# jeong0982/gkr

Hardware: AMD Instinct MI355X
Metric: BN254-Fr sumcheck field-ops/sec @ 2^20 vars (higher is better)
Workload: dtype u32x8

## Files before the change

gkr_amd/csrc/capi_internal.h:

```cpp
#pragma once
#include <hip/hip_runtime.h>
#include <sched.h>
#include <stdio.h>
#include <stdlib.h>
#include <string.h>

#include <algorithm>
#include <chrono>
#include <condition_variable>
#include <map>
#include <memory>
#include <mutex>
#include <string>
#include <thread>
#include <vector>

#include "../../include/gkr_amd.h"
#include "fr64.h"
#include "host_cpus.h"
#include "hostpool.h"
#include "kernels.h"
#include "options.h"
#include "gate_seg.h"
#include "keccak.h"
// ... 54 lines not shown
        }
        gkr::gkr_ifma_init(canon);
        return true;
    }();
    return ready;
}

inline gkr::h64::F host_multi_hash(const gkr::h64::F* arr, int n, const gkr::h64::F* cts) {
    static const bool adx = !gkr::process_switch("GKR_NO_ADX") && gkr::gkr_adx_available();
    if (!adx) return gkr::h64::mimc7_multi_hash(arr, n, cts, nullptr);
    gkr::h64::F out;
    gkr::gkr_adx_multi_hash(reinterpret_cast<const uint64_t(*)[4]>(arr), n, reinterpret_cast<const uint64_t(*)[4]>(cts), out.l);
    return out;
}

constexpr int kHashChunkMax = 16;
constexpr int kMaxLayerK = GKR_MAX_K_NEXT, kMaxLayerKi = GKR_MAX_K_I, kMaxDenseK = GKR_MAX_K_NEXT_DEVICE_TRANSCRIPT;
inline void ifma_hash_chunk(const uint64_t (*vec)[3][4], const uint32_t* ln, int count, uint64_t (*out)[4]) {
    if (count > 8)
        gkr::gkr_ifma_multi_hash16(vec, ln, 3, out);
    else
        gkr::gkr_ifma_multi_hash8(vec, ln, 3, out);
}
inline int hash_chunk_size(int tables, int threads, int help_share = 0) {
    const long long forced = gkr::opt(gkr::OPT_hash_chunk);
    if (forced == 8 || forced == 16) return (int)forced;
    if (help_share > 1 && tables <= 3 * help_share) return 1;
    return tables >= 32 * threads ? 16 : 8;
}

inline hipError_t device_malloc(void** p, size_t bytes) { return hipMalloc(p, bytes); }
inline hipError_t device_free(void* p) { return hipFree(p); }

inline int default_host_threads() {
    if (const int v = gkr::process_int("GKR_HOST_THREADS", 0); v >= 1) return v;
    int cpus = usable_cpus();
    int local = 1;
    if (const int ranks = gkr::process_int("LOCAL_WORLD_SIZE", 1); ranks > 0) local = ranks;
    const int share = cpus / local;
    int t = share >= 6 ? share - 2 : (share >= 3 ? share - 1 : share);
    if (t < 1) t = 1;
    if (t > 64) t = 64;
    return t;
}

inline Fr to_dev(const gkr_fr& x) {
    Fr f;
    memcpy(&f, &x, 32);
    return f;
}

// ... 104 lines not shown
    std::vector<std::unique_ptr<PreparedCircuit>> circuits;
    hipStream_t stream = nullptr;
    hipStream_t aux = nullptr;
    hipStream_t late = nullptr;
    hipStream_t chain = nullptr;
    std::vector<hipEvent_t> aux_events;
    Fr* d_cts = nullptr;
    int transcript = GKR_TRANSCRIPT_HOST;
    std::string err;
    int profile = 0;
    std::map<std::string, ProfileRow> prof;
    std::vector<PendingEvent> pending;
    std::vector<hipEvent_t> event_pool;
    char name[256] = {0};
    uint32_t ticket = 0;
    std::unique_ptr<gkr::SpinPool> pool;
    std::unique_ptr<gkr::SpinPool> solo_pool;
    std::unique_ptr<AsyncWorker> copier;
    std::unique_ptr<AsyncWorker> liner;
    void* mle_arrivals_zeroed = nullptr;
    void* arrivals_zeroed = nullptr;
    void* gate_arrive_zeroed = nullptr;
    bool crew_member = false;
    int help_share = 0;
    int rounds_ahead = 0;
    std::unique_ptr<ProveCrew, void (*)(ProveCrew*)> crew{nullptr, nullptr};
    std::map<std::string, std::pair<void*, size_t>> ws;
    std::map<std::string, std::pair<void*, size_t>> pinned;

    hipError_t workspace(const char* slot, size_t bytes, void** out) {
        auto& e = ws[slot];
        if (e.second < bytes) {
            if (e.first) (void)device_free(e.first);
            e.first = nullptr;
            e.second = 0;
            hipError_t rc = device_malloc(&e.first, bytes);
            if (rc != hipSuccess) return rc;
            e.second = bytes;
        }
        *out = e.first;
        return hipSuccess;
    }
    hipError_t pinned_host(const char* slot, size_t bytes, void** out) {
        auto& e = pinned[slot];
        if (e.second < bytes) {
            if (e.first) (void)hipHostFree(e.first);
            e.first = nullptr;
// ... 148 lines not shown
        if (_e != hipSuccess) return (ctx)->hip_fail(_e, #expr); \
    } while (0)


namespace gkr_host {


template <typename T>
struct DevBuf {
    T* p = nullptr;
    ~DevBuf() {
        if (p) (void)hipFree(p);
    }
    hipError_t alloc(size_t count) { return hipMalloc(reinterpret_cast<void**>(&p), count * sizeof(T)); }
};

struct ThreadTimeAccount {
    double own_pieces_us = 0, helped_us = 0, spin_us = 0;
};
inline thread_local ThreadTimeAccount t_account;
struct HostAccountTotals {
    std::atomic<uint64_t> own_ns{0}, helped_ns{0}, spin_ns{0}, rest_ns{0}, lent_ns{0}, lent_idle_ns{0}, calls{0}, wake_ns{0};
    std::atomic<uint64_t> pieces{0}, piece_ns{0}, piece_pass_ns{0}, lanes[17] = {};
    std::atomic<bool> on{false};
};
inline HostAccountTotals& host_account_totals() {
    static HostAccountTotals t;
    return t;
}
inline bool accounting_on() { return host_account_totals().on.load(std::memory_order_relaxed); }
inline void account_piece(int transcripts, double pass_us, double total_us) {
    HostAccountTotals& t = host_account_totals();
    t.pieces.fetch_add(1, std::memory_order_relaxed);
    t.piece_ns.fetch_add((uint64_t)(total_us * 1e3), std::memory_order_relaxed);
    t.piece_pass_ns.fetch_add((uint64_t)(pass_us * 1e3), std::memory_order_relaxed);
    t.lanes[transcripts < 1 ? 1 : (transcripts > 16 ? 16 : transcripts)].fetch_add(1, std::memory_order_relaxed);
}
inline double now_us_dbg() { return std::chrono::duration<double, std::micro>(std::chrono::steady_clock::now().time_since_epoch()).count(); }

inline bool help_enabled() {
    static const bool on = !gkr::process_switch("GKR_NO_HELP");
    return on;
}
static void run_pieces(gkr::SpinPool* pool, const std::function<bool()>* work, bool several, int priority = 0) {
    auto run = [&] {
        if (pool)
            pool->run_now(work);
        else
            while ((*work)()) {
            }
    };
    const bool dbg = gkr::debug_timing() || accounting_on();
    const double t0 = dbg ? now_us_dbg() : 0.0;
    if (several && help_enabled()) {
        gkr::HelpBoard::Posted posted(work, priority);
        run();
    } else {
        run();
    }
    if (dbg) t_account.own_pieces_us += now_us_dbg() - t0;
}

template <typename Rec>
inline int wait_records(gkr_ctx* ctx, const volatile Rec* recs, int count, uint32_t ticket) {
    const auto t0 = std::chrono::steady_clock::now();
    const bool help = help_enabled();
    auto last_progress = t0;
    for (int b = 0; b < count; ++b) {
        uint32_t spins = 0, helped = 0;
        while (__atomic_load_n(&recs[b].seq, __ATOMIC_ACQUIRE) != ticket) {
            const bool dbg = gkr::debug_timing() || accounting_on();
            const double th0 = dbg ? now_us_dbg() : 0.0;
            const bool did_help = help && gkr::HelpBoard::instance().help();
            if (!did_help) GKR_CPU_RELAX();
            if (dbg) (did_help ? t_account.helped_us : t_account.spin_us) += now_us_dbg() - th0;
            if (did_help ? (++helped & 0x3F) == 0 : (++spins & 0xFFFF) == 0) {
                hipError_t q = hipStreamQuery(ctx->stream);
                if (q != hipSuccess && q != hipErrorNotReady) return ctx->hip_fail(q, "stream failed while waiting for a round");
                if (std::chrono::steady_clock::now() - last_progress > std::chrono::seconds(30)) {
                    if (q == hipSuccess && __atomic_load_n(&recs[b].seq, __ATOMIC_ACQUIRE) == ticket) break;
                    return ctx->fail(GKR_ERR_HIP, "timed out waiting for the device to publish a round");
                }
            }
        }
        if (spins | helped) last_progress = std::chrono::steady_clock::now();
    }
    return GKR_OK;
}

constexpr int kMaxGroups = 32;
constexpr int kMleShardTailLog2 = 6;

#define WS(ctx, slot, type, count, ptr) \
    HIP_TRY(ctx, (ctx)->workspace(slot, (size_t)(count) * sizeof(type), reinterpret_cast<void**>(&(ptr))))

inline int mle_pass_rounds(int m, int n, int jmax) {
// ... 119 lines not shown
```

gkr_amd/csrc/capi_layer.hip:

```cpp
#include "capi_internal.h"

namespace gkr_host {

void host_prod_pass_scalar(const uint64_t* recs, size_t rec_row_words, int count, int J, const uint32_t (*vec_len)[16],
                                  uint64_t (*c2)[16][4], uint64_t (*lin)[16][4], uint64_t (*c0)[16][4], uint64_t (*r)[16][4],
                                  uint64_t* weights, size_t w_row_words) {
    using namespace gkr::h64;
    const F* cts = host_mimc_constants64();
    const F one_m = to_mont(F{{1, 0, 0, 0}});
    for (int k = 0; k < count; ++k) {
        F M[64], SY[8], rm[gkr::kProdMaxJ];
        const F* rec = reinterpret_cast<const F*>(recs + (size_t)k * rec_row_words);
        const int n = 1 << J;
        for (int a = 0; a < n; ++a) {
            for (int b = 0; b < n; ++b) M[a * 8 + b] = rec[a * 8 + b];
            SY[a] = rec[64 + a];
        }
        for (int t = 0; t < J; ++t) {
            const int half = 1 << (J - t - 1);
            F p00 = M[0], p01 = M[half], p10 = M[half * 8], p11 = M[half * 8 + half], s0 = SY[0], s1 = SY[half];
            for (int x = 1; x < half; ++x) {
                p00 = add(p00, M[x * 8 + x]);
                p01 = add(p01, M[x * 8 + half + x]);
                p10 = add(p10, M[(half + x) * 8 + x]);
// ... 261 lines not shown
            gkr::launch_gate_rows_wide(R.span, k_i, k, R.g->plan, R.gate_eq(), R.eq, R.A, R.M, R.lb, R.item_partials, R.gate_arrive, R.s, R.sets, R.plan_counts,
                                       R.wu ? &wfuse : nullptr);
            c_tables_done = R.wu != nullptr;
        } else
            c_tables_done = gkr::launch_gate_rows(R.span, k_i, k, R.g->offsets, R.g->cursor, R.g->list, R.e_hi, R.e_lo, R.kl, R.eq, R.A, R.M, R.lb, &R.g->segs,
                                                  R.seg_partials, R.s, R.shard ? nullptr : &fuse, R.sets);
    }
    if (R.shard)
        if (const int rc = xch.sum(R.A, R.M, R.wlen, nullptr, GKR_OK)) return rc;
    if (!c_tables_done) gkr::launch_prod_c_setup(R.Wb, jp, P.pw, R.A, R.M, R.X, R.Y, k, (uint32_t)R.wlen, batch, R.s);
    return GKR_OK;
}

struct HostPass {
    const LayerPinned* pin;
    int batch, k;
    bool ifma;
    gkr_fr* const* out_coeffs;
    uint32_t* const* out_len;
    gkr_fr* const* out_r;
    uint32_t J, round0, tail_m, tail_jp;
    bool on_host;
    int chunk;
    std::atomic<int> next{0};
};

static bool host_pass_piece(HostPass& hp) {
    const LayerPinned& P = *hp.pin;
    const int first = hp.next.fetch_add(hp.chunk, std::memory_order_relaxed);
    if (first >= hp.batch) return false;
    const int cnt = hp.batch - first < hp.chunk ? hp.batch - first : hp.chunk;
    uint64_t c2[gkr::kProdMaxJ][16][4], lin[gkr::kProdMaxJ][16][4], c0[gkr::kProdMaxJ][16][4], rr[gkr::kProdMaxJ][16][4];
    uint32_t vl[gkr::kProdMaxJ][16];
    const bool acct = accounting_on();
    const double tp0 = acct ? now_us_dbg() : 0.0;
    if (hp.on_host)
        for (int i = 0; i < cnt; ++i)
            host_tail_pass(reinterpret_cast<gkr::h64::F*>(P.tail + (size_t)(first + i) * 3 * P.tail_stride()), P.tail_stride(), hp.tail_m, hp.tail_jp,
                           reinterpret_cast<const gkr::h64::F*>(P.pw + (size_t)(first + i) * 8), hp.J, reinterpret_cast<gkr::h64::F*>(&P.prec[first + i].v[0]));
    for (uint32_t t = 0; t < hp.J; ++t)
        for (int i = 0; i < cnt; ++i) vl[t][i] = 2u + (P.dep[(size_t)(first + i) * 32 + (hp.round0 + t) % hp.k] ? 1u : 0u);
    (hp.ifma && cnt >= 3 ? gkr::gkr_ifma_prod_pass : host_prod_pass_scalar)(
        reinterpret_cast<const uint64_t*>(P.prec + first), sizeof(gkr::ProdPassRec) / 8, cnt, (int)hp.J, vl, c2, lin, c0, rr,
        reinterpret_cast<uint64_t*>(P.pw + (size_t)first * 8), 32);
    const double tp1 = acct ? now_us_dbg() : 0.0;
    for (int i = 0; i < cnt; ++i) {
        const int b = first + i;
        for (uint32_t t = 0; t < hp.J; ++t) {
            const uint32_t round = hp.round0 + t;
            gkr_fr* oc = hp.out_coeffs[b] + (size_t)round * 3;
            memset(&oc[0], 0, 32);
            if (vl[t][i] == 3) memcpy(&oc[0], c2[t][i], 32);
            memcpy(&oc[1], lin[t][i], 32);
// ... 48 lines not shown
            const bool on_host = tail_active;
            const bool exports = P.tail && !on_host && m - jp <= P.tail_log2 && rem > J;
            if (!on_host) {
                const uint32_t ticket = ++ctx->ticket;
                const double tl0 = dbg_sections ? now_us_dbg() : 0.0;
                {
                    Timed t(ctx, "layer_prod_pass", 0.0);
                    gkr::launch_prod_pass(Tw, Tx, Ty, m, jp, P.pw, J, d_ppart, (uint32_t)R.wlen, P.prec, ticket, (uint32_t)batch, R.s, d_arrivals, d_fold_plans,
                                          exports ? P.tail : nullptr, (uint32_t)P.tail_stride());
                }
                if (hipError_t le = hipGetLastError(); le != hipSuccess) {
                    rc = ctx->hip_fail(le, "launch of a layer pass");
                    break;
                }
                const double tl1 = dbg_sections ? now_us_dbg() : 0.0;
                rc = wait_records(ctx, P.prec, batch, ticket);
                if (dbg_sections) {
                    us_launch += tl1 - tl0;
                    us_wait += now_us_dbg() - tl1;
                }
                if (!rc) rc = xch.check();
                if (rc) break;
            }
            const int chunk = hash_chunk_size(batch, pool ? pool->workers() + 1 : 1, ctx->crew_member ? ctx->help_share : 0);
            HostPass hp{&P, batch, k, ifma, out_coeffs, out_len, out_r, J, round0, on_host ? tail_m : 0u, jp, on_host, chunk};
            const std::function<bool()> work = [&hp]() -> bool { return host_pass_piece(hp); };
            m -= jp;
            const double tw0 = dbg_sections ? now_us_dbg() : 0.0;
            run_pieces(pool, &work, batch > chunk, ctx->rounds_ahead + (int)(2 * k - round0));
            if (dbg_sections) us_pieces += now_us_dbg() - tw0;
            if (exports) tail_active = true;
            if (exports || on_host) tail_m = m;
            jp = J;
            round0 += J;
            rem -= J;
        }
    }
    session.close();
    if (dbg_sections)
        fprintf(stderr, "[gkr timing] layer k_i=%d k=%d batch=%d passes: %.0f us = launch calls %.0f + waiting for records %.0f + hashing pieces %.0f + c-phase set-up calls %.0f + other %.0f\n",
                R.k_i, k, batch, now_us_dbg() - t_passes0, us_launch, us_wait, us_pieces, us_phase1,
                now_us_dbg() - t_passes0 - us_launch - us_wait - us_pieces - us_phase1);
    return rc;
}

static int run_layer_gates(gkr_ctx* ctx, int batch, int k_i, int k, const uint8_t* d_gt, const uint32_t* d_l, const uint32_t* d_r, const gkr_fr* z,
                           const Fr* d_W, gkr_fr* const* out_coeffs, uint32_t* const* out_len, gkr_fr* const* out_r, const LayerShardArgs* shard,
                           GateLists* cached, const LayerGroup* group) {
    hipStream_t s = ctx->stream;
    const bool lists_fresh = !(cached && cached->ready);
    LayerRun R{ctx, s, batch, k_i, k, (size_t)1 << k, gkr::GateSpan{shard ? shard->gate_base : 0, shard ? shard->gate_count : (uint64_t)1 << k_i}};
    LayerPinned P;
// ... 382 lines not shown
```

gkr_amd/csrc/capi_mle_passes.hip:

```cpp
#include "capi_internal.h"

namespace gkr_host {

void host_pass_scalar(const uint64_t* sums, size_t sums_row_words, int count, int J, const uint32_t* final_len,
                             uint64_t (*c0)[16][4], uint64_t (*c1)[16][4], uint64_t (*r)[16][4], uint32_t (*len)[16],
                             uint64_t* weights, size_t w_row_words) {
    using gkr::h64::F;
    const F* cts = host_mimc_constants64();
    const F one_m = gkr::h64::to_mont(F{{1, 0, 0, 0}});
    for (int k = 0; k < count; ++k) {
        F S[gkr::kMleMaxSub], rm[gkr::kMlePassMaxRounds];
        memcpy(S, sums + (size_t)k * sums_row_words, sizeof(F) << J);
        for (int t = 0; t < J; ++t) {
            const int half = 1 << (J - t - 1);
            F lo = S[0], hi = S[half];
            for (int b = 1; b < half; ++b) {
                lo = gkr::h64::add(lo, S[b]);
                hi = gkr::h64::add(hi, S[half + b]);
            }
            const F d = gkr::h64::sub(hi, lo);
            const uint32_t ln = (final_len && t == J - 1) ? final_len[k] : (gkr::h64::is_zero(d) ? 1u : 2u);
            const F vec[2] = {d, lo};
            const F rc = host_multi_hash(vec + (2 - ln), (int)ln, cts);
            memcpy(c0[t][k], &lo, 32);
// ... 458 lines not shown
    void gather_tail(const Fr* rest, size_t stride, int m, int lp, int shard, Fr* d_tail) {
        hipStream_t s = ctx->stream;
        Timed t(ctx, "exchange", 0.0);
        gkr::launch_mle_gather_widen(rest, stride, (uint32_t)m, (uint32_t)lp, (uint32_t)shard, rc ? 1u : 0u, (uint32_t)batch, limbs(), s);
        const int arc = exchange->fn(exchange->user, ((size_t)batch << (m + lp)) * 8 + 8, static_cast<void*>(s));
        gkr::launch_mle_gather_narrow(limbs(), (uint32_t)(m + lp), (uint32_t)batch, d_tail, h_fail, s);
        ++exchanges;
        hook_failed(arc);
    }
    void rounds_chunk(int first, int J, int round0) {
        const int count = batch - first < 16 ? batch - first : 16;
        uint64_t c0[gkr::kMlePassMaxRounds][16][4], c1[gkr::kMlePassMaxRounds][16][4], r[gkr::kMlePassMaxRounds][16][4];
        uint32_t ln[gkr::kMlePassMaxRounds][16];
        (host_ifma_ready() && count >= 3 ? gkr::gkr_ifma_pass : host_pass_scalar)(
            reinterpret_cast<const uint64_t*>(T.h_rec[first].sums), sizeof(gkr::MleHostRecSub) / 8, count, J, nullptr, c0, c1, r, ln,
            reinterpret_cast<uint64_t*>(T.h_w + (size_t)first * gkr::kMleMaxSub), 4 * gkr::kMleMaxSub);
        for (int i = 0; i < count; ++i) {
            if (round0 == 0) dep_last[first + i] = T.h_rec[first + i].dep;
            for (int t = 0; t < J; ++t)
                write_round_output(out_coeffs, out_len, out_r, (size_t)(first + i) * n + round0 + t, c0[t][i], c1[t][i], ln[t][i], r[t][i]);
        }
    }
    void host_rounds(int J, int round0) {
        std::atomic<int> next{0};
        const std::function<bool()> work_fn = [&]() -> bool {
            const int first = next.fetch_add(16, std::memory_order_relaxed);
            if (first < batch) rounds_chunk(first, J, round0);
            return first < batch;
        };
        gkr::SpinPool::Session session(pool, nullptr);
        run_pieces(pool, &work_fn, batch > 16);
    }
    void pass(bool pass0, bool from_input, int m_src, int jin, int J, int round0) {
        const uint32_t ticket = ++ctx->ticket;
        if (!rc) {
            MlePassPolicy P;
            P.row = pass0 ? "mle_sub_sums" : "mle_multifold";
            if (pass0)
                queue_pass0(ctx, T, 0, batch, J, ticket, ctx->stream, P);
            else
                queue_fold(ctx, T, 0, batch, from_input, m_src, jin, J, ticket, ctx->stream, P);
            if (hipError_t le = hipGetLastError(); le != hipSuccess) rc = ctx->hip_fail(le, "launch of a sumcheck pass");
        }
        exchange_sums(J, ticket);
        if (!rc) rc = wait_records(ctx, T.h_rec, batch, ticket);
        if (!rc && some_rank_failed()) rc = ctx->fail(GKR_ERR_HIP, "another rank failed during the sumcheck");
        if (!rc) host_rounds(J, round0);
    }
};
}

}

extern "C" {
// ... 74 lines not shown
```

gkr_amd/csrc/capi_prove.hip:

```cpp
#include "capi_internal.h"

namespace gkr_host {

void mobius_msb(std::vector<gkr::h64::F>& c, int k) {
    const size_t n = (size_t)1 << k;
    for (int b = 0; b < k; ++b) {
        const size_t bit = (size_t)1 << (k - 1 - b);
        for (size_t i = 0; i < n; ++i)
            if (i & bit) c[i] = gkr::h64::sub(c[i], c[i ^ bit]);
    }
}

void line_restriction(const std::vector<gkr::h64::F>& vals, const std::vector<gkr::h64::F>& coeffs, int k, const gkr_fr* b,
                      const gkr_fr* c, gkr_fr* out, uint32_t* out_len) {
    using gkr::h64::F;
    const F zero = {{0, 0, 0, 0}};
    int maxdeg = 0;
    const size_t n = (size_t)1 << k;
    for (size_t mono = 0; mono < n; ++mono)
        if (!gkr::h64::is_zero(coeffs[mono])) {
            const int deg = __builtin_popcountll((unsigned long long)mono);
            if (deg > maxdeg) maxdeg = deg;
        }
    const size_t stride = (size_t)k + 1;
// ... 274 lines not shown
    std::vector<std::unique_ptr<PreparedCircuit>> fresh((size_t)n_members);
    struct DropFresh {
        gkr_ctx* ctx;
        std::vector<std::unique_ptr<PreparedCircuit>>& v;
        ~DropFresh() {
            bool any = false;
            for (auto& p : v) any |= (bool)p;
            if (any) (void)hipStreamSynchronize(ctx->stream);
            for (auto& p : v)
                if (p) p->release();
        }
    } drop_fresh{ctx, fresh};
    std::vector<uint64_t> hs((size_t)2 * n_members);
    {
        std::vector<HashSegment> segs;
        std::vector<size_t> first_seg((size_t)n_members + 1, 0);
        size_t total_bytes = 0;
        for (int m = 0; m < n_members; ++m) {
            circuit_hash_segments(members[m].circuit, segs);
            first_seg[(size_t)m + 1] = segs.size();
        }
        for (const HashSegment& sg : segs) total_bytes += sg.n;
        std::vector<uint64_t> seg_hashes(2 * segs.size());
        std::atomic<size_t> next{0};
        const std::function<bool()> work = [&]() -> bool {
            const size_t i = next.fetch_add(1, std::memory_order_relaxed);
            if (i >= segs.size()) return false;
            const size_t m = (size_t)(std::upper_bound(first_seg.begin(), first_seg.end(), i) - first_seg.begin()) - 1;
            hash_segment(segs[i], i - first_seg[m], &seg_hashes[2 * i], &seg_hashes[2 * i + 1]);
            return true;
        };
        gkr::SpinPool* hash_pool = (!ctx->crew_member && total_bytes >= ((size_t)2 << 20)) ? ctx->host_pool() : nullptr;
        gkr::SpinPool::Session session(hash_pool, nullptr);
        run_pieces(hash_pool, &work, segs.size() > (size_t)n_members);
        session.close();
        for (int m = 0; m < n_members; ++m)
            fold_segment_hashes(members[m].circuit->depth, &seg_hashes[2 * first_seg[m]], first_seg[(size_t)m + 1] - first_seg[m], &hs[2 * (size_t)m],
                                &hs[2 * (size_t)m + 1]);
    }
    for (int m = 0; m < n_members; ++m) {
        for (int e = 0; e < m && !pcs[m]; ++e)
            if (members[e].circuit == members[m].circuit) pcs[m] = pcs[e];
        if (pcs[m]) continue;
        rc = find_or_upload_circuit(ctx, members[m].circuit, hs[2 * (size_t)m], hs[2 * (size_t)m + 1], &pcs[m], fresh[m]);
        if (rc) return rc;
    }
    PreparedCircuit* pc = pcs[0];
    const bool any_fresh = [&] {
        for (auto& p : fresh)
            if (p) return true;
        return false;
    }();
    const double us_hash = us_since_entry();

    gkr::GateSet* d_sets = nullptr;
    std::vector<LayerGroup> groups;
    if (n_members > 1) {
// ... 17 lines not shown
                for (int half = 0; half < 2; ++half)
                    for (int w = 0; w < 8; ++w)
                        if (pcn.hdr[half][w] > groups[i].plan_counts.hdr[half][w]) groups[i].plan_counts.hdr[half][w] = pcn.hdr[half][w];
            }
            for (int b = 0; b < batch; ++b) {
                const PreparedCircuit* p = pcs[member_of[b]];
                const GateLists& gl = p->lists[i];
                h_sets[(size_t)i * batch + b] = gkr::GateSet{gl.offsets, gl.cursor, gl.list, gl.plan, p->gt[i], p->l[i], p->r[i], 0};
            }
        }
        gkr::launch_copy_words(h_sets, d_sets, n_sets * sizeof(gkr::GateSet) / 4, s);
    }

    std::vector<Fr*> dW(L + 1, nullptr);
    for (uint32_t i = 0; i <= L; ++i) {
        const std::string slot = "prove.W" + std::to_string(i);
        HIP_TRY(ctx, ctx->workspace(slot.c_str(), ((size_t)batch << c->k[i]) * sizeof(Fr), reinterpret_cast<void**>(&dW[i])));
    }
    constexpr size_t kKernelCopyLimit = (size_t)4 << 20, kGroupCopyLimit = (size_t)64 << 20;
    const size_t in_bytes = n_in * batch * sizeof(Fr);
    if (in_bytes <= (n_members > 1 ? kGroupCopyLimit : kKernelCopyLimit)) {
        gkr_fr* h_in = nullptr;
        HIP_TRY(ctx, ctx->pinned_host("prove.in", in_bytes, reinterpret_cast<void**>(&h_in)));
        std::atomic<int> next{0};
        const std::function<bool()> work = [&]() -> bool {
            const int m = next.fetch_add(1, std::memory_order_relaxed);
            if (m >= n_members) return false;
            memcpy(h_in + (size_t)first_of[m] * n_in, members[m].input_values, n_in * members[m].batch * sizeof(gkr_fr));
            return true;
        };
        run_pieces(nullptr, &work, n_members > 1 && in_bytes >= ((size_t)1 << 20));
        gkr::launch_copy_words(h_in, dW[L], in_bytes / 4, s);
    } else {
        for (int m = 0; m < n_members; ++m)
            HIP_TRY(ctx, hipMemcpyAsync(dW[L] + (size_t)first_of[m] * n_in, members[m].input_values, n_in * members[m].batch * sizeof(Fr), hipMemcpyHostToDevice, s));
    }
    uint32_t* d_in_flag = nullptr;
    uint32_t h_in_flag = 0;
    if (check_on_device) {
        WS(ctx, "prove.inflag", uint32_t, 1, d_in_flag);
        HIP_TRY(ctx, hipMemsetAsync(d_in_flag, 0, 4, s));
        gkr::launch_check_canonical(dW[L], n_in * (size_t)batch, d_in_flag, s);
    }
    for (int i = (int)L - 1; i >= 0; --i)
        gkr::launch_layer_eval(1u << c->k[i], pc->gt[i], pc->l[i], pc->r[i], dW[i + 1], dW[i], (uint32_t)batch, 1u << c->k[i + 1], s,
                               n_members > 1 ? groups[i].d_sets : nullptr);
    HIP_TRY(ctx, hipGetLastError());
    HIP_TRY(ctx, ctx->aux_stream(1));
    hipStream_t side = ctx->aux;
    std::vector<F> hW_big[2];
    struct SideDrain {
        hipStream_t st;
        ~SideDrain() {
            if (st) (void)hipStreamSynchronize(st);
// ... 180 lines not shown
                gkr::launch_line_restriction(Wn, (uint32_t)k, reinterpret_cast<const Fr*>(lines), d_lr, d_lrdeg, bcm, qdst, qlen_dst, (uint32_t)batch, aux);
            }
        }
        auto finish = [&](int b) {
            const gkr_fr* sr = srp[b];
            const gkr_fr* b_star = sr;
            const gkr_fr* c_star = sr + k;
            const gkr_fr r_star = sr[2 * k - 1];
            outs[b].r[i] = r_star;
            F rs;
            memcpy(&rs, &r_star, 32);
            rs = gkr::h64::to_mont(rs);
            gkr_fr* zn = outs[b].z + z_off + k_i;
            for (int j = 0; j < k; ++j) {
                F bj, cj;
                memcpy(&bj, &b_star[j], 32);
                memcpy(&cj, &c_star[j], 32);
                const F v = gkr::h64::add(bj, gkr::h64::mont_mul(gkr::h64::sub(cj, bj), rs));
                memcpy(&zn[j], &v, 32);
                memcpy(&z_next[(size_t)b * k + j], &v, 32);
            }
        };
        {
            std::atomic<int> next{0};
            const std::function<bool()> work = [&]() -> bool {
                const int b = next.fetch_add(1, std::memory_order_relaxed);
                if (b >= batch) return false;
                finish(b);
                return true;
            };
            gkr::SpinPool::Session session(pool, nullptr);
            run_pieces(pool, &work, batch > 1);
        }
        if (dbg_pb)
            fprintf(stderr, "[gkr timing] prove layer %u: sumcheck %.0f us, q / z on the host %.0f us (since entry of the hand-off: %.0f us)\n", i,
                    std::chrono::duration<double, std::micro>(tl1 - tl0).count(),
                    std::chrono::duration<double, std::micro>(std::chrono::steady_clock::now() - tl1).count(),
                    std::chrono::duration<double, std::micro>(std::chrono::steady_clock::now() - tpb0).count());
        z_cur.swap(z_next);
        row_off += (size_t)2 * k;
        q_off += (size_t)k + 1;
        z_off += (size_t)k_i;
    }
    {
        HIP_TRY(ctx, hipGetLastError());
        copier.finish();
        liner.finish();
        HIP_TRY(ctx, hipStreamSynchronize(ctx->aux));
        if (h_in_flag) return ctx->fail(GKR_ERR_NON_CANONICAL, "input value >= r");
        for (int b = 0; b < batch; ++b) {
            if (members[member_of[b]].require_zero_output && !gkr::h64::is_zero(hW0_first ? hW0_first[b] : hW[0][(size_t)b << c->k[0]]))
                return ctx->fail(GKR_ERR_INVALID, "output 0 is not zero (convert.rs:838 asserts d_values[0] == 0)");
            std::vector<F> co;
            if (!coeffs_done[0]) {
                co.assign(hW[0] + ((size_t)b << c->k[0]), hW[0] + ((size_t)(b + 1) << c->k[0]));
// ... 52 lines not shown
    return GKR_OK;
}

static int prove_batch_impl(gkr_ctx* ctx, const gkr_circuit_desc* c, const gkr_fr* input_values, int batch, int require_zero_output,
                            gkr_proof_buf* outs) {
    gkr_prove_item one{c, input_values, batch, require_zero_output, outs, 0};
    return prove_group_impl(ctx, &one, 1);
}

int gkr_prove(gkr_ctx* ctx, const gkr_circuit_desc* c, const gkr_fr* input_values, int require_zero_output,
              gkr_proof_buf* out) {
    if (!ctx) return GKR_ERR_INVALID;
    return prove_batch_impl(ctx, c, input_values, 1, require_zero_output, out);
}

int gkr_prove_batch(gkr_ctx* ctx, const gkr_circuit_desc* c, const gkr_fr* input_values, int batch, int require_zero_output,
                    gkr_proof_buf* outs) {
    if (!ctx) return GKR_ERR_INVALID;
    return prove_batch_impl(ctx, c, input_values, batch, require_zero_output, outs);
}

static void crew_prove_items(ProveCrew* crew, ProveCrew::Member* m) {
    if (accounting_on()) host_account_totals().wake_ns.fetch_add((uint64_t)((now_us_dbg() - crew->t_call_us) * 1e3), std::memory_order_relaxed);
    m->ctx->help_share = crew->units->empty() ? 1 : (crew->active + (int)crew->units->size() - 1) / (int)crew->units->size();
    for (int u : m->items) {
        const std::vector<int>& unit = (*crew->units)[u];
        auto prove_one = [&](int idx) {
            gkr_prove_item& it = crew->items[idx];
            if (!it.circuit || !it.input_values || !it.outs) {
                it.status = m->ctx->fail(GKR_ERR_INVALID, "null pointer in a prove item");
                return;
            }
            it.status = prove_batch_impl(m->ctx, it.circuit, it.input_values, it.batch, it.require_zero_output, it.outs);
        };
        if (unit.size() == 1) {
            prove_one(unit[0]);
            continue;
        }
        std::vector<gkr_prove_item> group;
        for (int idx : unit) group.push_back(crew->items[idx]);
        const int rc = prove_group_impl(m->ctx, group.data(), (int)group.size());
        if (rc == GKR_OK) {
            for (int idx : unit) crew->items[idx].status = GKR_OK;
        } else {
            for (int idx : unit) prove_one(idx);
        }
    }
// ... 213 lines not shown
```

gkr_amd/csrc/gkr_capi.hip:

```cpp
#include "capi_internal.h"


extern "C" {

const char* gkr_strerror(int status) {
    switch (status) {
        case GKR_OK: return "ok";
        case GKR_ERR_INVALID: return "invalid argument";
        case GKR_ERR_NON_CANONICAL: return "field element is not canonical (>= r)";
        case GKR_ERR_NO_DEVICE: return "no gfx950 device available";
        case GKR_ERR_HIP: return "HIP runtime error";
        case GKR_ERR_NOMEM: return "out of memory";
        case GKR_ERR_DEGENERATE: return "degenerate sumcheck (v == 0)";
        case GKR_ERR_UNSUPPORTED: return "R1CS shape the reference's compiler does not support";
        default: return "unknown status";
    }
}

const char* gkr_version(void) { return "gkr_amd 0.1 (gfx950)"; }

int gkr_ctx_create(int device_id, gkr_ctx** out) {
    if (!out) return GKR_ERR_INVALID;
    *out = nullptr;
    int count = 0;
// ... 109 lines not shown
            drop_cache(child);
            child->options = ctx->options;
        }
    if (prev_device >= 0) (void)hipSetDevice(prev_device);
    return GKR_OK;
}

int gkr_ctx_set_host_threads(gkr_ctx* ctx, int threads) {
    if (!ctx || threads < 0 || threads > 256) return GKR_ERR_INVALID;
    if (threads != ctx->host_threads) {
        ctx->pool.reset();
        ctx->host_threads = threads;
    }
    return GKR_OK;
}

long gkr_host_help_while(const volatile int32_t* busy) {
    if (!busy) return 0;
    long pieces = 0;
    unsigned idle = 0;
    const bool account = accounting_on();
    const double t0 = account ? now_us_dbg() : 0.0;
    double lent_us = 0;
    while (__atomic_load_n(busy, __ATOMIC_ACQUIRE) != 0) {
        const double th = account ? now_us_dbg() : 0.0;
        if (help_enabled() && gkr::HelpBoard::instance().help()) {
            if (account) lent_us += now_us_dbg() - th;
            ++pieces;
            idle = 0;
            continue;
        }
        GKR_CPU_RELAX();
        if (++idle > 4096) {
            std::this_thread::yield();
            idle = 0;
        }
    }
    if (account) {
        HostAccountTotals& tot = host_account_totals();
        const double all = now_us_dbg() - t0;
        tot.lent_ns.fetch_add((uint64_t)(lent_us * 1e3), std::memory_order_relaxed);
        tot.lent_idle_ns.fetch_add((uint64_t)((all > lent_us ? all - lent_us : 0) * 1e3), std::memory_order_relaxed);
    }
    return pieces;
}

int gkr_host_accounting(int enable) {
    HostAccountTotals& tot = host_account_totals();
    if (enable) {
        tot.own_ns = 0;
        tot.helped_ns = 0;
        tot.spin_ns = 0;
        tot.rest_ns = 0;
        tot.lent_ns = 0;
        tot.lent_idle_ns = 0;
        tot.calls = 0;
        tot.wake_ns = 0;
        tot.pieces = 0;
        tot.piece_ns = 0;
        tot.piece_pass_ns = 0;
        for (auto& l : tot.lanes) l = 0;
    }
    tot.on.store(enable != 0, std::memory_order_relaxed);
    return GKR_OK;
}

int gkr_host_accounting_read(double* out_us, size_t count) {
    if (!out_us || count < 7) return GKR_ERR_INVALID;
    if (count >= 8) out_us[7] = host_account_totals().wake_ns.load() * 1e-3;
    const HostAccountTotals& tot = host_account_totals();
    out_us[0] = tot.own_ns.load() * 1e-3;
    out_us[1] = tot.helped_ns.load() * 1e-3;
    out_us[2] = tot.spin_ns.load() * 1e-3;
    out_us[3] = tot.rest_ns.load() * 1e-3;
    out_us[4] = tot.lent_ns.load() * 1e-3;
    out_us[5] = tot.lent_idle_ns.load() * 1e-3;
    out_us[6] = (double)tot.calls.load();
    if (count >= 28) {
        out_us[8] = (double)tot.pieces.load();
        out_us[9] = tot.piece_ns.load() * 1e-3;
        out_us[10] = tot.piece_pass_ns.load() * 1e-3;
        for (int n = 1; n <= 16; ++n) out_us[10 + n] = (double)tot.lanes[n].load();
        out_us[27] = 0.0;
    }
    return GKR_OK;
}

int gkr_ctx_device_name(const gkr_ctx* ctx, char* buf, size_t len) {
    if (!ctx || !buf || !len) return GKR_ERR_INVALID;
    snprintf(buf, len, "%s", ctx->name);
    return GKR_OK;
}

int gkr_ctx_profile(gkr_ctx* ctx, int enable) {
    if (!ctx) return GKR_ERR_INVALID;
    ctx->profile = enable < 0 ? 0 : (enable > 2 ? 2 : enable);
    return GKR_OK;
}

int gkr_ctx_profile_get(gkr_ctx* ctx, const char* kernel, uint64_t* launches, double* total_ms, double* bytes) {
    if (!ctx || !kernel) return GKR_ERR_INVALID;
    ctx->drain_events();
    auto it = ctx->prof.find(kernel);
    ProfileRow r = it == ctx->prof.end() ? ProfileRow() : it->second;
    if (launches) *launches = r.launches;
    if (total_ms) *total_ms = r.total_ms;
    if (bytes) *bytes = r.bytes;
// ... 503 lines not shown
```

gkr_amd/csrc/hostpool.h:

```cpp
#pragma once
#include <atomic>
#include <condition_variable>
#include <functional>
#include <mutex>
#include <thread>
#include <vector>

#if defined(__x86_64__)
#include <immintrin.h>
#define GKR_CPU_RELAX() _mm_pause()
#else
#define GKR_CPU_RELAX() ((void)0)
#endif

namespace gkr {

class HelpBoard {
   public:
    static HelpBoard& instance() {
        static HelpBoard board;
        return board;
    }
    int post(const std::function<bool()>* work, int priority = 0) {
        for (int i = 0; i < kSlots; ++i) {
            const std::function<bool()>* expected = nullptr;
            if (slots_[i].job.compare_exchange_strong(expected, work, std::memory_order_seq_cst)) {
                slots_[i].priority.store(priority, std::memory_order_relaxed);
                posted_.fetch_add(1, std::memory_order_seq_cst);
                return i;
            }
        }
        return -1;
    }
    void retire(int slot) {
        if (slot < 0) return;
        slots_[slot].job.store(nullptr, std::memory_order_seq_cst);
        posted_.fetch_sub(1, std::memory_order_seq_cst);
        while (slots_[slot].inside.load(std::memory_order_seq_cst) != 0) GKR_CPU_RELAX();
    }
    bool help() {
        if (posted_.load(std::memory_order_acquire) == 0) return false;
        const int start = next_.fetch_add(1, std::memory_order_relaxed);
        uint64_t tried = 0;
        for (;;) {
            int best = -1, best_prio = 0;
            for (int n = 0; n < kSlots; ++n) {
                const int i = (start + n) % kSlots;
                if ((tried >> i) & 1u) continue;
                if (slots_[i].job.load(std::memory_order_acquire) == nullptr) continue;
                const int pr = slots_[i].priority.load(std::memory_order_relaxed);
                if (best < 0 || pr > best_prio) {
                    best = i;
                    best_prio = pr;
                }
            }
            if (best < 0) return false;
            tried |= (uint64_t)1 << best;
            Slot& sl = slots_[best];
            sl.inside.fetch_add(1, std::memory_order_seq_cst);
            const std::function<bool()>* job = sl.job.load(std::memory_order_seq_cst);
            const bool did = job && (*job)();
            sl.inside.fetch_sub(1, std::memory_order_seq_cst);
            if (did) return true;
        }
    }

    class Posted {
       public:
        explicit Posted(const std::function<bool()>* work, int priority = 0) : slot_(HelpBoard::instance().post(work, priority)) {}
        ~Posted() { HelpBoard::instance().retire(slot_); }
        Posted(const Posted&) = delete;
        Posted& operator=(const Posted&) = delete;

       private:
        int slot_;
    };

   private:
    static constexpr int kSlots = 64;
    struct alignas(64) Slot {
        std::atomic<const std::function<bool()>*> job{nullptr};
        std::atomic<int> inside{0};
        std::atomic<int> priority{0};
    };
    Slot slots_[kSlots];
    std::atomic<int> posted_{0};
    std::atomic<unsigned> next_{0};
};

class SpinPool {
   public:
    explicit SpinPool(int workers) {
        for (int i = 0; i < workers; ++i) threads_.emplace_back([this] { worker(); });
    }
    ~SpinPool() {
        {
            std::lock_guard<std::mutex> g(mu_);
            stop_.store(true);
        }
        cv_.notify_all();
        for (auto& t : threads_) t.join();
    }
    int workers() const { return (int)threads_.size(); }

    void begin_session(const std::function<bool()>* try_work) {
        {
            std::lock_guard<std::mutex> g(mu_);
            fn_ = try_work;
            session_.fetch_add(1, std::memory_order_release);
        }
// ... 84 lines not shown
```

Measured before the change: 454.5 billion.

## Rework help board into indexed piece slots with adaptive crew chunk sizing

Replaces the std::function-based help board with indexed job slots. Each slot hands out pieces through a generation-tagged atomic cursor, tracks completions with a done counter, and keeps an occupancy bitmask, so helpers claim pieces directly instead of calling closures that each hold their own atomic counter. It also tracks free helper threads and open pieces, and uses them to choose the hash chunk size for crew members from an estimated pass cost, replacing the fixed help_share heuristic. The aim is lower contention and overhead when distributing host work and better load balance, at the cost of more complex lock-free bookkeeping in which a retire or exhaustion race could cause stalls.

```diff
diff --git a/gkr_amd/csrc/capi_internal.h b/gkr_amd/csrc/capi_internal.h
--- a/gkr_amd/csrc/capi_internal.h
+++ b/gkr_amd/csrc/capi_internal.h
@@ -100,11 +100,27 @@
     else
         gkr::gkr_ifma_multi_hash8(vec, ln, 3, out);
 }
-inline int hash_chunk_size(int tables, int threads, int help_share = 0) {
+inline int hash_chunk_size(int tables, int threads) {
     const long long forced = gkr::opt(gkr::OPT_hash_chunk);
     if (forced == 8 || forced == 16) return (int)forced;
-    if (help_share > 1 && tables <= 3 * help_share) return 1;
     return tables >= 32 * threads ? 16 : 8;
+}
+inline int crew_chunk_size(int tables) {
+    const long long forced = gkr::opt(gkr::OPT_hash_chunk);
+    if (forced == 8 || forced == 16) return (int)forced;
+    const gkr::HelpBoard& board = gkr::HelpBoard::instance();
+    const long long idle = (long long)board.free_threads() - board.open_pieces();
+    const long long threads = 1 + (idle > 0 ? idle : 0);
+    auto pass_cost = [&](int chunk) {
+        const int widest = tables < chunk ? tables : chunk;
+        const long long piece = widest <= 2 ? 5 * widest : (widest <= 8 ? 10 : 13);
+        const long long pieces = (tables + chunk - 1) / chunk;
+        return (pieces + threads - 1) / threads * piece;
+    };
+    int best = 16;
+    for (const int chunk : {8, 1})
+        if (pass_cost(chunk) < pass_cost(best)) best = chunk;
+    return best;
 }
 
 inline hipError_t device_malloc(void** p, size_t bytes) { return hipMalloc(p, bytes); }
@@ -255,7 +271,6 @@
     void* arrivals_zeroed = nullptr;
     void* gate_arrive_zeroed = nullptr;
     bool crew_member = false;
-    int help_share = 0;
     int rounds_ahead = 0;
     std::unique_ptr<ProveCrew, void (*)(ProveCrew*)> crew{nullptr, nullptr};
     std::map<std::string, std::pair<void*, size_t>> ws;
@@ -450,6 +465,7 @@
 struct HostAccountTotals {
     std::atomic<uint64_t> own_ns{0}, helped_ns{0}, spin_ns{0}, rest_ns{0}, lent_ns{0}, lent_idle_ns{0}, calls{0}, wake_ns{0};
     std::atomic<uint64_t> pieces{0}, piece_ns{0}, piece_pass_ns{0}, lanes[17] = {};
+    std::atomic<uint64_t> retire_wait_ns{0};
     std::atomic<bool> on{false};
 };
 inline HostAccountTotals& host_account_totals() {
@@ -470,36 +486,49 @@
     static const bool on = !gkr::process_switch("GKR_NO_HELP");
     return on;
 }
-static void run_pieces(gkr::SpinPool* pool, const std::function<bool()>* work, bool several, int priority = 0) {
-    auto run = [&] {
-        if (pool)
-            pool->run_now(work);
-        else
-            while ((*work)()) {
-            }
-    };
+static void run_pieces(gkr::SpinPool* pool, const gkr::HelpJob& job, bool share) {
+    if (job.count < 1) return;
     const bool dbg = gkr::debug_timing() || accounting_on();
     const double t0 = dbg ? now_us_dbg() : 0.0;
-    if (several && help_enabled()) {
-        gkr::HelpBoard::Posted posted(work, priority);
-        run();
-    } else {
-        run();
-    }
-    if (dbg) t_account.own_pieces_us += now_us_dbg() - t0;
+    gkr::HelpBoard& board = gkr::HelpBoard::instance();
+    gkr::HelpBoard::Slot own;
+    gkr::HelpBoard::Slot* slot = share && help_enabled() ? board.post(job) : nullptr;
+    if (!slot) {
+        slot = &own;
+        gkr::HelpBoard::open(own, job);
+    }
+    if (pool) {
+        const std::function<bool()> work = [&board, slot]() -> bool { return board.take(*slot); };
+        pool->run_now(&work);
+    } else
+        while (board.take(*slot)) {
+        }
+    const double t1 = dbg ? now_us_dbg() : 0.0;
+    board.retire(*slot);
+    if (dbg) {
+        const double t2 = now_us_dbg();
+        t_account.own_pieces_us += t2 - t0;
+        if (accounting_on()) host_account_totals().retire_wait_ns.fetch_add((uint64_t)((t2 - t1) * 1e3), std::memory_order_relaxed);
+    }
+}
+template <typename Fn>
+static void run_indexed_pieces(gkr::SpinPool* pool, Fn& piece, int count, bool share, int priority = 0) {
+    run_pieces(pool, gkr::HelpJob{[](void* f, int i) -> bool { (*static_cast<Fn*>(f))(i); return true; }, &piece, count, priority}, share);
 }
 
 template <typename Rec>
 inline int wait_records(gkr_ctx* ctx, const volatile Rec* recs, int count, uint32_t ticket) {
     const auto t0 = std::chrono::steady_clock::now();
     const bool help = help_enabled();
+    gkr::HelpBoard::FreeThread free_mark;
     auto last_progress = t0;
     for (int b = 0; b < count; ++b) {
         uint32_t spins = 0, helped = 0;
         while (__atomic_load_n(&recs[b].seq, __ATOMIC_ACQUIRE) != ticket) {
             const bool dbg = gkr::debug_timing() || accounting_on();
             const double th0 = dbg ? now_us_dbg() : 0.0;
-            const bool did_help = help && gkr::HelpBoard::instance().help();
+            if (help) free_mark.enter();
+            const bool did_help = help && gkr::HelpBoard::instance().help(true);
             if (!did_help) GKR_CPU_RELAX();
             if (dbg) (did_help ? t_account.helped_us : t_account.spin_us) += now_us_dbg() - th0;
             if (did_help ? (++helped & 0x3F) == 0 : (++spins & 0xFFFF) == 0) {
diff --git a/gkr_amd/csrc/capi_layer.hip b/gkr_amd/csrc/capi_layer.hip
--- a/gkr_amd/csrc/capi_layer.hip
+++ b/gkr_amd/csrc/capi_layer.hip
@@ -307,13 +307,13 @@
     uint32_t J, round0, tail_m, tail_jp;
     bool on_host;
     int chunk;
-    std::atomic<int> next{0};
+    int pieces() const { return (batch + chunk - 1) / chunk; }
 };
 
-static bool host_pass_piece(HostPass& hp) {
+static bool host_pass_piece(void* pass, int piece) {
+    const HostPass& hp = *static_cast<const HostPass*>(pass);
     const LayerPinned& P = *hp.pin;
-    const int first = hp.next.fetch_add(hp.chunk, std::memory_order_relaxed);
-    if (first >= hp.batch) return false;
+    const int first = piece * hp.chunk;
     const int cnt = hp.batch - first < hp.chunk ? hp.batch - first : hp.chunk;
     uint64_t c2[gkr::kProdMaxJ][16][4], lin[gkr::kProdMaxJ][16][4], c0[gkr::kProdMaxJ][16][4], rr[gkr::kProdMaxJ][16][4];
     uint32_t vl[gkr::kProdMaxJ][16];
@@ -408,12 +408,11 @@
                 if (!rc) rc = xch.check();
                 if (rc) break;
             }
-            const int chunk = hash_chunk_size(batch, pool ? pool->workers() + 1 : 1, ctx->crew_member ? ctx->help_share : 0);
+            const int chunk = ctx->crew_member ? crew_chunk_size(batch) : hash_chunk_size(batch, pool ? pool->workers() + 1 : 1);
             HostPass hp{&P, batch, k, ifma, out_coeffs, out_len, out_r, J, round0, on_host ? tail_m : 0u, jp, on_host, chunk};
-            const std::function<bool()> work = [&hp]() -> bool { return host_pass_piece(hp); };
             m -= jp;
             const double tw0 = dbg_sections ? now_us_dbg() : 0.0;
-            run_pieces(pool, &work, batch > chunk, ctx->rounds_ahead + (int)(2 * k - round0));
+            run_pieces(pool, gkr::HelpJob{&host_pass_piece, &hp, hp.pieces(), ctx->rounds_ahead + (int)(2 * k - round0)}, batch > chunk);
             if (dbg_sections) us_pieces += now_us_dbg() - tw0;
             if (exports) tail_active = true;
             if (exports || on_host) tail_m = m;
diff --git a/gkr_amd/csrc/capi_mle_passes.hip b/gkr_amd/csrc/capi_mle_passes.hip
--- a/gkr_amd/csrc/capi_mle_passes.hip
+++ b/gkr_amd/csrc/capi_mle_passes.hip
@@ -504,14 +504,9 @@
         }
     }
     void host_rounds(int J, int round0) {
-        std::atomic<int> next{0};
-        const std::function<bool()> work_fn = [&]() -> bool {
-            const int first = next.fetch_add(16, std::memory_order_relaxed);
-            if (first < batch) rounds_chunk(first, J, round0);
-            return first < batch;
-        };
+        auto chunk = [&](int i) { rounds_chunk(16 * i, J, round0); };
         gkr::SpinPool::Session session(pool, nullptr);
-        run_pieces(pool, &work_fn, batch > 16);
+        run_indexed_pieces(pool, chunk, (batch + 15) / 16, batch > 16);
     }
     void pass(bool pass0, bool from_input, int m_src, int jin, int J, int round0) {
         const uint32_t ticket = ++ctx->ticket;
diff --git a/gkr_amd/csrc/capi_prove.hip b/gkr_amd/csrc/capi_prove.hip
--- a/gkr_amd/csrc/capi_prove.hip
+++ b/gkr_amd/csrc/capi_prove.hip
@@ -320,17 +320,14 @@
         }
         for (const HashSegment& sg : segs) total_bytes += sg.n;
         std::vector<uint64_t> seg_hashes(2 * segs.size());
-        std::atomic<size_t> next{0};
-        const std::function<bool()> work = [&]() -> bool {
-            const size_t i = next.fetch_add(1, std::memory_order_relaxed);
-            if (i >= segs.size()) return false;
+        auto hash_one = [&](int piece) {
+            const size_t i = (size_t)piece;
             const size_t m = (size_t)(std::upper_bound(first_seg.begin(), first_seg.end(), i) - first_seg.begin()) - 1;
             hash_segment(segs[i], i - first_seg[m], &seg_hashes[2 * i], &seg_hashes[2 * i + 1]);
-            return true;
         };
         gkr::SpinPool* hash_pool = (!ctx->crew_member && total_bytes >= ((size_t)2 << 20)) ? ctx->host_pool() : nullptr;
         gkr::SpinPool::Session session(hash_pool, nullptr);
-        run_pieces(hash_pool, &work, segs.size() > (size_t)n_members);
+        run_indexed_pieces(hash_pool, hash_one, (int)segs.size(), segs.size() > (size_t)n_members);
         session.close();
         for (int m = 0; m < n_members; ++m)
             fold_segment_hashes(members[m].circuit->depth, &seg_hashes[2 * first_seg[m]], first_seg[(size_t)m + 1] - first_seg[m], &hs[2 * (size_t)m],
@@ -394,14 +391,8 @@
     if (in_bytes <= (n_members > 1 ? kGroupCopyLimit : kKernelCopyLimit)) {
         gkr_fr* h_in = nullptr;
         HIP_TRY(ctx, ctx->pinned_host("prove.in", in_bytes, reinterpret_cast<void**>(&h_in)));
-        std::atomic<int> next{0};
-        const std::function<bool()> work = [&]() -> bool {
-            const int m = next.fetch_add(1, std::memory_order_relaxed);
-            if (m >= n_members) return false;
-            memcpy(h_in + (size_t)first_of[m] * n_in, members[m].input_values, n_in * members[m].batch * sizeof(gkr_fr));
-            return true;
-        };
-        run_pieces(nullptr, &work, n_members > 1 && in_bytes >= ((size_t)1 << 20));
+        auto stage = [&](int m) { memcpy(h_in + (size_t)first_of[m] * n_in, members[m].input_values, n_in * members[m].batch * sizeof(gkr_fr)); };
+        run_indexed_pieces(nullptr, stage, n_members, n_members > 1 && in_bytes >= ((size_t)1 << 20));
         gkr::launch_copy_words(h_in, dW[L], in_bytes / 4, s);
     } else {
         for (int m = 0; m < n_members; ++m)
@@ -628,15 +619,8 @@
             }
         };
         {
-            std::atomic<int> next{0};
-            const std::function<bool()> work = [&]() -> bool {
-                const int b = next.fetch_add(1, std::memory_order_relaxed);
-                if (b >= batch) return false;
-                finish(b);
-                return true;
-            };
             gkr::SpinPool::Session session(pool, nullptr);
-            run_pieces(pool, &work, batch > 1);
+            run_indexed_pieces(pool, finish, batch, batch > 1);
         }
         if (dbg_pb)
             fprintf(stderr, "[gkr timing] prove layer %u: sumcheck %.0f us, q / z on the host %.0f us (since entry of the hand-off: %.0f us)\n", i,
@@ -735,7 +719,6 @@
 
 static void crew_prove_items(ProveCrew* crew, ProveCrew::Member* m) {
     if (accounting_on()) host_account_totals().wake_ns.fetch_add((uint64_t)((now_us_dbg() - crew->t_call_us) * 1e3), std::memory_order_relaxed);
-    m->ctx->help_share = crew->units->empty() ? 1 : (crew->active + (int)crew->units->size() - 1) / (int)crew->units->size();
     for (int u : m->items) {
         const std::vector<int>& unit = (*crew->units)[u];
         auto prove_one = [&](int idx) {
diff --git a/gkr_amd/csrc/gkr_capi.hip b/gkr_amd/csrc/gkr_capi.hip
--- a/gkr_amd/csrc/gkr_capi.hip
+++ b/gkr_amd/csrc/gkr_capi.hip
@@ -155,9 +155,11 @@
     const bool account = accounting_on();
     const double t0 = account ? now_us_dbg() : 0.0;
     double lent_us = 0;
+    gkr::HelpBoard::FreeThread free_mark;
+    if (help_enabled()) free_mark.enter();
     while (__atomic_load_n(busy, __ATOMIC_ACQUIRE) != 0) {
         const double th = account ? now_us_dbg() : 0.0;
-        if (help_enabled() && gkr::HelpBoard::instance().help()) {
+        if (help_enabled() && gkr::HelpBoard::instance().help(true)) {
             if (account) lent_us += now_us_dbg() - th;
             ++pieces;
             idle = 0;
@@ -193,6 +195,7 @@
         tot.piece_ns = 0;
         tot.piece_pass_ns = 0;
         for (auto& l : tot.lanes) l = 0;
+        tot.retire_wait_ns = 0;
     }
     tot.on.store(enable != 0, std::memory_order_relaxed);
     return GKR_OK;
@@ -216,6 +219,7 @@
         for (int n = 1; n <= 16; ++n) out_us[10 + n] = (double)tot.lanes[n].load();
         out_us[27] = 0.0;
     }
+    if (count >= 29) out_us[28] = tot.retire_wait_ns.load() * 1e-3;
     return GKR_OK;
 }
 
diff --git a/gkr_amd/csrc/hostpool.h b/gkr_amd/csrc/hostpool.h
--- a/gkr_amd/csrc/hostpool.h
+++ b/gkr_amd/csrc/hostpool.h
@@ -1,6 +1,7 @@
 #pragma once
 #include <atomic>
 #include <condition_variable>
+#include <cstdint>
 #include <functional>
 #include <mutex>
 #include <thread>
@@ -15,56 +16,130 @@
 
 namespace gkr {
 
+struct HelpJob {
+    bool (*run)(void* ctx, int piece) = nullptr;
+    void* ctx = nullptr;
+    int count = 0;
+    int priority = 0;
+};
+
 class HelpBoard {
    public:
+    static constexpr int kSlots = 64;
+    static constexpr int kMaxPieces = 1 << 24;
+    struct alignas(64) Slot {
+        std::atomic<uint64_t> cursor{0};
+        std::atomic<uint32_t> done{0};
+        std::atomic<uint32_t> exhausted{0};
+        std::atomic<int> count{0}, priority{0};
+        bool (*run)(void*, int) = nullptr;
+        void* ctx = nullptr;
+        int index = -1;
+    };
     static HelpBoard& instance() {
         static HelpBoard board;
         return board;
     }
-    int post(const std::function<bool()>* work, int priority = 0) {
-        for (int i = 0; i < kSlots; ++i) {
-            const std::function<bool()>* expected = nullptr;
-            if (slots_[i].job.compare_exchange_strong(expected, work, std::memory_order_seq_cst)) {
-                slots_[i].priority.store(priority, std::memory_order_relaxed);
-                posted_.fetch_add(1, std::memory_order_seq_cst);
-                return i;
-            }
-        }
-        return -1;
-    }
-    void retire(int slot) {
-        if (slot < 0) return;
-        slots_[slot].job.store(nullptr, std::memory_order_seq_cst);
-        posted_.fetch_sub(1, std::memory_order_seq_cst);
-        while (slots_[slot].inside.load(std::memory_order_seq_cst) != 0) GKR_CPU_RELAX();
-    }
-    bool help() {
-        if (posted_.load(std::memory_order_acquire) == 0) return false;
-        const int start = next_.fetch_add(1, std::memory_order_relaxed);
-        uint64_t tried = 0;
+    HelpBoard() {
+        for (int i = 0; i < kSlots; ++i) slots_[i].index = i;
+    }
+    static void open(Slot& s, const HelpJob& job) {
+        s.run = job.run;
+        s.ctx = job.ctx;
+        s.count.store(job.count, std::memory_order_relaxed);
+        s.priority.store(job.priority, std::memory_order_relaxed);
+        s.done.store(0, std::memory_order_relaxed);
+        const uint64_t gen = (s.cursor.load(std::memory_order_relaxed) >> 32) + 1;
+        s.cursor.store(gen << 32, std::memory_order_release);
+    }
+    Slot* post(const HelpJob& job) {
+        if (job.count < 1 || job.count > kMaxPieces) return nullptr;
+        uint64_t occ = occ_.load(std::memory_order_relaxed);
+        uint64_t bit;
+        do {
+            if (!~occ) return nullptr;
+            bit = ~occ & (occ + 1);
+        } while (!occ_.compare_exchange_weak(occ, occ | bit, std::memory_order_acq_rel, std::memory_order_relaxed));
+        Slot& s = slots_[__builtin_ctzll(bit)];
+        open_.fetch_add(job.count, std::memory_order_relaxed);
+        open(s, job);
+        return &s;
+    }
+    bool take(Slot& s) {
+        uint64_t c = s.cursor.load(std::memory_order_acquire);
         for (;;) {
-            int best = -1, best_prio = 0;
-            for (int n = 0; n < kSlots; ++n) {
-                const int i = (start + n) % kSlots;
-                if ((tried >> i) & 1u) continue;
-                if (slots_[i].job.load(std::memory_order_acquire) == nullptr) continue;
-                const int pr = slots_[i].priority.load(std::memory_order_relaxed);
-                if (best < 0 || pr > best_prio) {
-                    best = i;
+            if (!((c >> 32) & 1) || (uint32_t)c >= (uint32_t)s.count.load(std::memory_order_relaxed)) return false;
+            if (s.exhausted.load(std::memory_order_relaxed) == (uint32_t)(c >> 32)) return false;
+            if (s.cursor.compare_exchange_weak(c, c + 1, std::memory_order_acq_rel, std::memory_order_acquire)) break;
+        }
+        return run_claimed(s, c);
+    }
+    void retire(Slot& s) {
+        const uint64_t gen = s.cursor.load(std::memory_order_relaxed) >> 32;
+        const uint64_t last = s.cursor.exchange((gen + 1) << 32, std::memory_order_acq_rel);
+        const uint32_t claimed = (uint32_t)last, count = (uint32_t)s.count.load(std::memory_order_relaxed);
+        if (s.index >= 0 && claimed < count) open_.fetch_sub((long long)(count - claimed), std::memory_order_relaxed);
+        while (s.done.load(std::memory_order_acquire) != claimed) GKR_CPU_RELAX();
+        if (s.index >= 0) occ_.fetch_and(~((uint64_t)1 << s.index), std::memory_order_release);
+    }
+    bool help(bool counted = false) {
+        if (open_.load(std::memory_order_acquire) <= 0) return false;
+        static thread_local unsigned rot = 0;
+        for (int attempt = 0; attempt < 3; ++attempt) {
+            const uint64_t occ = occ_.load(std::memory_order_acquire);
+            const unsigned r = rot & 63u;
+            Slot* best = nullptr;
+            uint64_t best_c = 0;
+            int best_prio = 0;
+            for (uint64_t m = (occ >> r) | (r ? occ << (64u - r) : 0); m; m &= m - 1) {
+                Slot& s = slots_[((unsigned)__builtin_ctzll(m) + r) & 63u];
+                const uint64_t c = s.cursor.load(std::memory_order_acquire);
+                if (!((c >> 32) & 1) || (uint32_t)c >= (uint32_t)s.count.load(std::memory_order_relaxed)) continue;
+                if (s.exhausted.load(std::memory_order_relaxed) == (uint32_t)(c >> 32)) continue;
+                const int pr = s.priority.load(std::memory_order_relaxed);
+                if (!best || pr > best_prio) {
+                    best = &s;
+                    best_c = c;
                     best_prio = pr;
                 }
             }
-            if (best < 0) return false;
-            tried |= (uint64_t)1 << best;
-            Slot& sl = slots_[best];
-            sl.inside.fetch_add(1, std::memory_order_seq_cst);
-            const std::function<bool()>* job = sl.job.load(std::memory_order_seq_cst);
-            const bool did = job && (*job)();
-            sl.inside.fetch_sub(1, std::memory_order_seq_cst);
+            if (!best) return false;
+            if (!best->cursor.compare_exchange_strong(best_c, best_c + 1, std::memory_order_acq_rel, std::memory_order_relaxed)) continue;
+            ++rot;
+            if (counted) free_.fetch_sub(1, std::memory_order_relaxed);
+            const bool did = run_claimed(*best, best_c);
+            if (counted) free_.fetch_add(1, std::memory_order_relaxed);
             if (did) return true;
         }
-    }
-
+        return false;
+    }
+    int free_threads() const { return free_.load(std::memory_order_relaxed); }
+    long long open_pieces() const { return open_.load(std::memory_order_relaxed); }
+
+    class FreeThread {
+       public:
+        FreeThread() = default;
+        ~FreeThread() {
+            if (on_) HelpBoard::instance().free_.fetch_sub(1, std::memory_order_relaxed);
+        }
+        FreeThread(const FreeThread&) = delete;
+        FreeThread& operator=(const FreeThread&) = delete;
+        void enter() {
+            if (!on_) HelpBoard::instance().free_.fetch_add(1, std::memory_order_relaxed);
+            on_ = true;
+        }
+
+       private:
+        bool on_ = false;
+    };
+
+    int post(const std::function<bool()>* work, int priority = 0) {
+        Slot* s = post(HelpJob{&call_function, const_cast<std::function<bool()>*>(work), kMaxPieces, priority});
+        return s ? s->index : -1;
+    }
+    void retire(int slot) {
+        if (slot >= 0) retire(slots_[slot]);
+    }
     class Posted {
        public:
         explicit Posted(const std::function<bool()>* work, int priority = 0) : slot_(HelpBoard::instance().post(work, priority)) {}
@@ -77,15 +152,18 @@
     };
 
    private:
-    static constexpr int kSlots = 64;
-    struct alignas(64) Slot {
-        std::atomic<const std::function<bool()>*> job{nullptr};
-        std::atomic<int> inside{0};
-        std::atomic<int> priority{0};
-    };
+    static bool call_function(void* ctx, int) { return (*static_cast<const std::function<bool()>*>(ctx))(); }
+    bool run_claimed(Slot& s, uint64_t c) {
+        if (s.index >= 0) open_.fetch_sub(1, std::memory_order_relaxed);
+        const bool did = s.run(s.ctx, (int)(uint32_t)c);
+        if (!did) s.exhausted.store((uint32_t)(c >> 32), std::memory_order_relaxed);
+        s.done.fetch_add(1, std::memory_order_release);
+        return did;
+    }
     Slot slots_[kSlots];
-    std::atomic<int> posted_{0};
-    std::atomic<unsigned> next_{0};
+    alignas(64) std::atomic<uint64_t> occ_{0};
+    alignas(64) std::atomic<long long> open_{0};
+    alignas(64) std::atomic<int> free_{0};
 };
 
 class SpinPool {
```

Result: no change. 453.0 billion (-0.3%).
